# voutcn/megahit

Measured on AMD Instinct MI355X. Metric: M (k+1)-mer edges sorted+counted/sec, sdbg_build k=21, higher is better.
Workload: dtype u32; 1 GPU; read2sdbg (S1+S2) k=21 m=2 no mercy, 10000000 synthetic 150 bp PE reads per GPU (BASELINE configs[1]), inputs resident in HBM, outputs left in HBM; reads_per_gpu=10000000, edges_per_gpu=1290000000, k=21, min_count=2, parallelism=1 GPU, s1_items=1330000000, s2_items=117381042, sdbg_records=59857080

## Files before the change

megahit_amd/csrc/mhx_internal.h:

```cpp
#pragma once
#include <hip/hip_runtime.h>

#include <cstdint>
#include <cstdio>
#include <cstring>
#include <functional>
#include <map>
#include <stdexcept>
#include <string>
#include <vector>

#include "../../include/mhx.h"

namespace mhx {

struct OnesweepLaunch;
void set_error(const char *fmt, ...);

struct Error : std::runtime_error {
  explicit Error(const std::string &s) : std::runtime_error(s) {}
};

#define MHX_HIP(expr)                                                                          \
  do {                                                                                         \
// ... 93 lines not shown
    b.used = bytes;
    return b;
  }
  void prof_begin(const char *name, double bytes);
  void prof_end();
  void prof_collect();
};

#define MHX_LAUNCH(ctx, name, bytes, ...) \
  do {                                    \
    (ctx)->prof_begin(name, bytes);       \
    __VA_ARGS__;                          \
    MHX_HIP(hipGetLastError());           \
    (ctx)->prof_end();                    \
  } while (0)

namespace mhx {

struct SortPass {
  int shift;
  int bits;
  int shift2 = 0;
  int bits2 = 0;
  int prev_lo = -1;
};
struct SortPrep {
  const void *buf = nullptr;
  uint64_t n = 0;
  int hist_passes = 0;
  uint64_t hist_sig = 0;
  std::function<void(const OnesweepLaunch &)> gen;
  uint64_t gen_slots = 0;
  bool gen_var = false;
};
uint32_t *radix_sort(mhx_ctx *c, uint32_t *buf_a, uint32_t *buf_b, uint64_t n, int stride, int key_words,
                     const std::vector<SortPass> &passes, SortPrep *prep = nullptr);
uint32_t *sort_whole_key(mhx_ctx *c, uint32_t *buf_a, uint32_t *buf_b, uint64_t n, int stride, int key_words,
                         const std::vector<SortPass> &passes, SortPrep *prep = nullptr);
std::vector<SortPass> make_passes(int key_words, int lo_bit, int hi_bit);
bool sort_takes_generated_first_pass(const mhx_ctx *c, uint64_t n, int stride, const std::vector<SortPass> &passes);
uint64_t passes_signature(const std::vector<SortPass> &ps);
uint32_t *kmsort_exact(mhx_ctx *c, uint32_t *buf_a, uint32_t *buf_b, uint64_t n, int S, int key_words, SortPrep *prep = nullptr);

void exclusive_scan_u32_u64(mhx_ctx *c, const uint32_t *in, uint64_t *out, uint64_t n, uint64_t *d_total);
void exclusive_scan_u64(mhx_ctx *c, const uint64_t *in, uint64_t *out, uint64_t n, uint64_t *d_total);
void find_group_heads(mhx_ctx *c, const uint32_t *items, uint64_t n, int stride, int cmp_bits,
                      uint64_t *heads, uint64_t *d_count);
uint64_t count_group_heads(mhx_ctx *c, const uint32_t *items, uint64_t n, int stride, int cmp_bits);

struct DigitSpec;
DigitSpec spec_of_pass(const SortPass &ps, int key_words);
std::vector<SortPass> make_passes_ranges(int key_words, const std::vector<std::pair<int, int>> &ranges);
void emit_sdbg(mhx_ctx *c, const uint32_t *sorted, uint64_t n_items, int S, int kw, uint32_t k, int is_seq, mhx_sdbg_result *out, int compact_bits = 0);

void partition_by_owner(mhx_ctx *c, const uint32_t *a, uint32_t *b, uint64_t n, int stride, const uint8_t *lut, int n_parts,
                        uint64_t *counts);
uint64_t s1_extract(mhx_ctx *c, uint32_t k, bool compact, SortPrep *prep, bool defer_items = false, bool filter_in_gen = false);
bool s1_compact(const mhx_ctx *c, uint32_t k, int want_mercy);
bool s1_rank_tagged(const mhx_ctx *c, uint32_t k);
int s1_stride(uint32_t k, bool compact);
struct S1Sources {
  int n = 0;
  std::vector<const uint32_t *> ptr;
  std::vector<uint64_t> count;
  uint32_t *spare = nullptr;
  int pbits = 16;
};
constexpr int kSkmBatch = 8;
constexpr int kSkmSrcMax = 8;
struct SkmFront {
  int n_src;
  const uint4 *src[kSkmSrcMax];
  const uint64_t *src_bounds[kSkmSrcMax];
// ... 138 lines not shown
```

megahit_amd/csrc/s1_skm.hip:

```cpp
#include <cstring>

#include "s1_shared.h"

namespace mhx {

constexpr int kSkmC = 8;
constexpr int kSkmW = 10;
constexpr int kSkmNM = kSkmC + kSkmW - 1;
constexpr int kSkmMinBinBits = 16, kSkmMaxBinBits = 20;

__device__ __forceinline__ uint32_t skm_mix(uint32_t c) {
  uint32_t h = c * 0x9E3779B1u;
  return h ^ (h >> 15);
}
__device__ __forceinline__ uint32_t skm_mix2(uint32_t c) {
  uint32_t h = c * 0x9E3779B1u;
  h ^= h >> 15;
  return h * 0x85EBCA6Bu;
}
__device__ __forceinline__ uint32_t skm_bin_of(uint32_t minh) {
  return (minh ^ (minh >> 16)) * 0x7FEB352Du;
}

template <int NT, int J, bool VAR, bool COUNT = false>
__global__ __launch_bounds__(NT) void k_skm_make(const uint32_t *__restrict__ seq, const uint64_t *__restrict__ start, uint32_t L, uint32_t bpr, uint64_t n_blocks,
                                                 int k, int bin_bits, uint32_t bin_lo, uint32_t bin_hi, int count_items, uint64_t pos_base,
                                                 unsigned long long *__restrict__ hp, uint4 *__restrict__ out, unsigned long long cap,
                                                 unsigned long long *__restrict__ cursor, uint32_t *__restrict__ err, unsigned long long *__restrict__ digit_hist) {
  __shared__ uint32_t sm_scan[NT / kWave + 1];
  __shared__ unsigned long long s_base;
  __shared__ uint32_t dh[3][256];
  __shared__ uint32_t lbin[J * kSkmC][NT];
  __shared__ uint32_t hpl[2][12];
  const int tid = threadIdx.x;
  if (tid < 24) hpl[tid / 12][tid % 12] = 0;
  for (int i = tid; i < 768; i += NT) dh[i >> 8][i & 255] = 0;
  __syncthreads();
  const bool third_digit = bin_bits > 16;
  const int M = k + 1 - (kSkmW - 1);
  const uint32_t mmask = (1u << (2 * M)) - 1u;
  const int K1 = k + 1;
  const unsigned bin_sh = 32u - (unsigned)bin_bits;
  unsigned long long items = 0;
  uint32_t hp_n[2] = {0, 0};
  unsigned long long hp_p[2] = {~0ull, ~0ull};
  for (uint64_t it = blockIdx.x; it * (uint64_t)(NT * J) < n_blocks; it += gridDim.x) {
    uint64_t Wv[J], pos0[J];
    uint32_t smask[J], emask[J];
    uint32_t bflag[J];
#pragma unroll
    for (int j = 0; j < J; ++j) {
      const uint64_t b = it * (uint64_t)(NT * J) + (uint64_t)j * NT + tid;
      smask[j] = 0;
      emask[j] = 0;
      bflag[j] = 0;
      Wv[j] = 0;
      pos0[j] = 0;
      if (b < n_blocks) {
        const uint64_t r = b / bpr;
        const uint32_t q0 = (uint32_t)(b - r * bpr) * kSkmC;
        uint64_t base;
        uint32_t nwin;
        if constexpr (VAR) {
          base = start[r];
          const uint64_t len_r = start[r + 1] - base;
          nwin = len_r >= (uint64_t)K1 ? (uint32_t)(len_r - k) : 0u;
          if (q0 == 0 && nwin && count_items) items += nwin + (COUNT ? 0 : 4);
        } else {
          base = r * L;
// ... 45 lines not shown
                    const unsigned prev_raw = q0 + w == 0 ? kSentinel
                                              : (w == 0 ? (unsigned)((seq[(a - 1) >> 4] >> (30 - 2 * (unsigned)((a - 1) & 15))) & 3u) : (unsigned)(W >> (64 - 2 * w)) & 3u);
                    const unsigned next_raw = q0 + w + 1 == nwin ? kSentinel : (unsigned)(W >> (62 - 2 * (w + K1))) & 3u;
                    const unsigned pv = strand ? comp_or_sentinel(next_raw) : prev_raw, nx = strand ? comp_or_sentinel(prev_raw) : next_raw;
                    atomicAdd(&hpl[cls][0], 1u);
                    if (pv < 4) atomicAdd(&hpl[cls][1 + pv], 1u);
                    if (nx < 4) atomicAdd(&hpl[cls][5 + nx], 1u);
                  } else {
                    ++hp_n[cls];
                    hp_p[cls] = min(hp_p[cls], pos_base + a + (uint64_t)w);
                  }
                }
            }
          }
#pragma unroll
          for (int w = 0; w < kSkmC; ++w)
            if ((uint32_t)w < n_here && !((hm >> w) & 1u) && bins[w] >= bin_lo && bins[w] < bin_hi) km |= 1u << w;
#pragma unroll
          for (int w = 0; w < kSkmC; ++w)
            if (((km >> w) & 1u) && (w == 0 || !((km >> (w - 1)) & 1u) || bins[w] != bins[w > 0 ? w - 1 : 0])) sm |= 1u << w;
          smask[j] = sm;
          emask[j] = km & ((sm >> 1) | ~(km >> 1));
          if constexpr (COUNT) {
            const uint64_t pb = a > 0 ? (uint64_t)((seq[(a - 1) >> 4] >> (30 - 2 * (unsigned)((a - 1) & 15))) & 3u) : 0ull;
            Wv[j] = (W >> 2) | (pb << 62);
            bflag[j] = (q0 == 0 ? 1u : 0u) | (q0 + n_here == nwin ? 2u : 0u) | (n_here << 2);
          } else {
            Wv[j] = W;
          }
          pos0[j] = pos_base + a;
        }
      }
    }
    uint32_t cnt = 0;
#pragma unroll
    for (int j = 0; j < J; ++j) cnt += (uint32_t)__builtin_popcount(smask[j]);
    uint32_t total = 0;
    const uint32_t excl = block_exclusive_sum<uint32_t, NT>(cnt, sm_scan, &total);
    if (tid == 0) s_base = total ? atomicAdd(cursor, (unsigned long long)total) : 0ull;
    __syncthreads();
    const unsigned long long base = s_base;
    if (base + total > cap) {
      if (tid == 0) atomicOr(err, 1u);
      return;
    }
    unsigned long long at = base + excl;
#pragma unroll
    for (int j = 0; j < J; ++j) {
      uint32_t sm = smask[j], em = emask[j];
      while (sm) {
        const int rs = __builtin_ctz(sm), re = __builtin_ctz(em);
        sm &= sm - 1;
        em &= em - 1;
        const int len = re - rs + 1;
        const uint32_t run_bin = lbin[j * kSkmC + rs][tid];
        const uint64_t p = pos0[j] + (uint64_t)rs;
        if constexpr (COUNT) {
          const uint64_t bases = (Wv[j] << (2 * rs)) & (~0ull << (64 - 2 * (K1 + len + 1)));
          const uint32_t n_blk = bflag[j] >> 2;
          const uint32_t fl = ((bflag[j] & 1u) && rs == 0 ? 16u : 0u) | ((bflag[j] & 2u) && (uint32_t)(re + 1) == n_blk ? 8u : 0u);
          out[at++] = make_uint4((run_bin << 8) | ((uint32_t)(p >> 32) << 28) | ((uint32_t)(len - 1) << 5) | fl, (uint32_t)(bases >> 32), (uint32_t)bases, (uint32_t)p);
        } else {
        const uint64_t bases = ((Wv[j] << (2 * rs)) & (~0ull << (64 - 2 * (K1 + len - 1)))) | (uint64_t)(len - 1);
        out[at++] = make_uint4((run_bin << 8) | ((uint32_t)(p >> 32) << 28), (uint32_t)(bases >> 32), (uint32_t)bases, (uint32_t)p);
        }
        atomicAdd(&dh[0][run_bin & 255u], 1u);
        atomicAdd(&dh[1][(run_bin >> 8) & 255u], 1u);
        if (third_digit) atomicAdd(&dh[2][run_bin >> 16], 1u);
      }
    }
  }
  if constexpr (VAR) {
    items = wave_sum(items);
    if ((tid & (kWave - 1)) == 0 && items) atomicAdd(cursor + 3, items);
  }
  if constexpr (COUNT) {
    __syncthreads();
    if (hp && count_items && tid < 24 && hpl[tid / 12][tid % 12]) atomicAdd(hp + 8 + (tid / 12) * 16 + (tid % 12), (unsigned long long)hpl[tid / 12][tid % 12]);
  }
  if (!COUNT && hp && count_items) {
#pragma unroll
    for (int x = 0; x < 2; ++x) {
      const uint32_t n_w = wave_sum(hp_n[x]);
      if (n_w) {
        unsigned long long pmin = hp_p[x];
#pragma unroll
        for (int d = kWave / 2; d > 0; d >>= 1) pmin = min(pmin, (unsigned long long)__shfl_xor((long long)pmin, d, kWave));
        if ((tid & (kWave - 1)) == 0) {
          atomicAdd(hp + x, (unsigned long long)n_w);
          atomicMin(hp + 2 + x, pmin);
        }
      }
    }
  }
  __syncthreads();
  for (int i = tid; i < 768; i += NT)
    if (dh[i >> 8][i & 255]) atomicAdd(&digit_hist[i], (unsigned long long)dh[i >> 8][i & 255]);
}

__global__ void k_skm_hp_publish(const unsigned long long *__restrict__ hp, int k, uint32_t m, uint8_t *__restrict__ solid_bytes,
                                 unsigned long long *__restrict__ hist, uint2 *__restrict__ agg_items, uint64_t *__restrict__ agg_cursor, int agg) {
  if (threadIdx.x || blockIdx.x) return;
// ... 914 lines not shown

bool s1_skm_dist_applies(const mhx_ctx *c, uint32_t k, uint32_t m) {
  const SeqSet &s = c->seqs;
  if (!c->opt("s1_skm", 1) || !c->opt("dist_skm", 1) || !c->global_bases || c->n_parts > kSkmSrcMax || c->filter_on || c->accumulate) return false;
  if (k < 19 || k > 22 || m < 1 || m > 2 || (c->global_bases >> 36)) return false;
  if (!s.n_seqs || s.max_len < k + 1) return false;
  if (!s.fixed_len && (double)s.n_bases * 100.0 < (double)c->opt("s1_var_min_fill", 50) * (double)s.n_seqs * s.max_len) return false;
  if (getenv("MHX_S1_MARK") || !c->opt("dist_sparse_marks", 1)) return false;
  return s1_skm_passes(c, k) == 1;
}

int s1_skm_passes(const mhx_ctx *c, uint32_t k) {
  const SeqSet &s = c->seqs;
  if (const long long f = c->opt("s1_skm_passes", 0)) return (int)std::min<long long>(64, std::max<long long>(1, f));
  const uint64_t n_win = s.n_bases > s.n_seqs * (uint64_t)k ? s.n_bases - s.n_seqs * (uint64_t)k : 0;
  const double need = (double)n_win * (double)std::max<long long>(c->opt("s1_skm_cap_pct", 36), 1) / 100.0 * 32.0;
  const double budget = (double)std::max<long long>(c->opt("s1_skm_pass_gb", 48), 1) * 1e9;
  return (int)std::min(64.0, std::max(1.0, std::ceil(need / budget)));
}

bool s1_skm_front(mhx_ctx *c, uint32_t k, SkmFront *f, int pass, int n_passes, int bin_bits_agreed, bool for_count) {
  SeqSet &s = c->seqs;
  hipStream_t st = c->stream;
  const bool var = s.fixed_len == 0;
  const uint32_t L = var ? s.max_len : s.fixed_len, bpr = (L - k + kSkmC - 1) / kSkmC;
  const uint64_t n_blocks = s.n_seqs * (uint64_t)bpr;
  const uint64_t n_win = var ? (s.n_bases > s.n_seqs * (uint64_t)k ? s.n_bases - s.n_seqs * (uint64_t)k : 0) : s.n_seqs * (uint64_t)(L - k);
  const uint64_t cap_all = n_win * (uint64_t)std::max<long long>(c->opt("s1_skm_cap_pct", 36), 1) / 100;
  const uint64_t cap = std::max<uint64_t>(n_passes > 1 ? cap_all / n_passes + cap_all / n_passes * 15 / 100 : cap_all, 1u << 16);
  int bin_bits = kSkmMinBinBits;
  while (bin_bits < kSkmMaxBinBits && (double)n_win * 0.29 / (double)(1ull << bin_bits) > 8192.0) ++bin_bits;
  if (const long long fb = c->opt("s1_skm_bin_bits", 0)) bin_bits = (int)std::min<long long>(kSkmMaxBinBits, std::max<long long>(8, fb));
  if (bin_bits_agreed > 0) bin_bits = bin_bits_agreed;
  uint4 *buf_a = c->ws("items_a", cap * 16 + 64).as<uint4>();
  uint4 *buf_b = c->ws("items_b", cap * 16 + 64).as<uint4>();
  unsigned long long *cursor = c->ws("skm_cursor", 64).as<unsigned long long>();
  uint32_t *err = reinterpret_cast<uint32_t *>(cursor + 1);
  uint32_t *max_bin = err + 1;
  MHX_HIP(hipMemsetAsync(cursor, 0, 64, st));
  std::vector<SortPass> passes;
  for (int lo = 0; lo < bin_bits; lo += 8) passes.push_back(SortPass{8 + lo, std::min(8, bin_bits - lo), 0, 0, 0});
  unsigned long long *pre_hist = c->ws("sort_pre_hist", (size_t)kMaxFusedPasses * 256 * 8).as<unsigned long long>();
  MHX_HIP(hipMemsetAsync(pre_hist, 0, (size_t)3 * 256 * 8, st));
  constexpr int NT = 512, J = 2;
  const uint64_t cus = c->n_cus > 0 ? (uint64_t)c->n_cus : 256;
  const unsigned grid = (unsigned)std::min<uint64_t>(div_ceil(n_blocks, (uint64_t)NT * J), cus * 8);
  const uint32_t n_bins = 1u << bin_bits;
  const uint32_t bin_lo = (uint32_t)((uint64_t)n_bins * pass / n_passes), bin_hi = (uint32_t)((uint64_t)n_bins * (pass + 1) / n_passes);
  unsigned long long *hp = nullptr;
  if (!c->global_bases && c->opt("s1_skm_hp", 1)) {
    hp = c->ws("skm_hp", 512).as<unsigned long long>();
    if (pass == 0) {
      unsigned long long init[48] = {0};
      init[2] = init[3] = ~0ull;
      MHX_HIP(hipMemcpyAsync(hp, init, sizeof init, hipMemcpyHostToDevice, st));
      MHX_HIP(hipStreamSynchronize(st));
    }
  }
#define MHX_MAKE(VARV, COUNTV)                                                                                                                                   \
  hipLaunchKernelGGL((k_skm_make<NT, J, VARV, COUNTV>), dim3(grid), dim3(NT), 0, st, s.words.as<uint32_t>(), s.start.as<uint64_t>(), L, bpr, n_blocks, (int)k, \
                     bin_bits, bin_lo, bin_hi, pass == 0 ? 1 : 0, c->pos_base, hp, buf_a, (unsigned long long)cap, cursor, err, pre_hist)
  MHX_LAUNCH(c, for_count ? "count_skm_make" : "s1_skm_make", (double)s.n_bases / 4 + (double)n_win * 16 / 3.5, {
    if (var && for_count) MHX_MAKE(true, true);
    else if (var) MHX_MAKE(true, false);
    else if (for_count) MHX_MAKE(false, true);
    else MHX_MAKE(false, false);
  });
#undef MHX_MAKE
  unsigned long long h[4] = {0, 0, 0, 0};
  std::vector<unsigned long long> h_dh(passes.size() * 256);
  MHX_HIP(hipMemcpyAsync(h, cursor, 32, hipMemcpyDeviceToHost, st));
  MHX_HIP(hipMemcpyAsync(h_dh.data(), pre_hist, h_dh.size() * 8, hipMemcpyDeviceToHost, st));
  MHX_HIP(hipStreamSynchronize(st));
  f->n_records = 0;
  f->hp = hp;
  if ((uint32_t)h[1] != 0 || h[0] > cap) return false;
  const uint64_t n = h[0];
  {
    const uint64_t n_bins_pass = std::max<uint64_t>(1, ((1ull << bin_bits) + n_passes - 1) / n_passes);
    const uint64_t limit = std::max<uint64_t>((uint64_t)c->opt("s1_skm_max_bin", 1 << 16), 16 * (n / n_bins_pass + 1));
    bool all = n > 0;
    uint64_t smallest_excess = ~0ull;
    for (size_t p = 0; p < passes.size() && all; ++p) {
      const uint64_t vals = 1ull << passes[p].bits;
      uint64_t mx = 0;
      for (uint64_t d = 0; d < vals; ++d) mx = std::max<uint64_t>(mx, h_dh[p * 256 + d]);
      const uint64_t mean = n / std::max<uint64_t>(1, (p + 1 == passes.size() && n_passes > 1) ? std::max<uint64_t>(1, vals / n_passes) : vals);
      const uint64_t excess = mx > mean ? mx - mean : 0;
      smallest_excess = std::min(smallest_excess, excess);
      all = excess >= limit + limit / 2;
    }
    if (all) {
      f->n_records = n;
      f->max_bin = (uint32_t)std::min<uint64_t>(smallest_excess, 0xFFFFFFFFu);
      return false;
    }
  }
  SortPrep prep;
  prep.buf = buf_a;
  prep.n = n;
  prep.hist_passes = (int)passes.size();
  prep.hist_sig = passes_signature(passes);
  uint32_t *sorted = radix_sort(c, reinterpret_cast<uint32_t *>(buf_a), reinterpret_cast<uint32_t *>(buf_b), n, 4, 1, passes, &prep);
  uint64_t *bounds = c->ws("s1_bucket_bounds", ((size_t)n_bins + 1) * 8 + 64).as<uint64_t>();
  MHX_LAUNCH(c, "s1_skm_bounds", (double)n_bins * 8 * 30,
             hipLaunchKernelGGL(k_skm_bounds, dim3((n_bins + 1 + 255) / 256), dim3(256), 0, st, reinterpret_cast<const uint4 *>(sorted), n, n_bins, bounds, max_bin));
  uint32_t h_max = 0;
  MHX_HIP(hipMemcpyAsync(&h_max, max_bin, 4, hipMemcpyDeviceToHost, st));
  MHX_HIP(hipStreamSynchronize(st));
  f->n_src = 1;
  f->src[0] = reinterpret_cast<const uint4 *>(sorted);
  f->src_bounds[0] = bounds;
  f->spare = sorted == reinterpret_cast<uint32_t *>(buf_a) ? reinterpret_cast<uint32_t *>(buf_b) : reinterpret_cast<uint32_t *>(buf_a);
  f->spare_bytes = cap * 16;
  f->n_records = n;
  f->n_windows = n_win;
  if (pass == 0) f->n_items = var ? h[3] : s.n_seqs * (uint64_t)(L - k + (for_count ? 0 : 4));
  f->n_bins = n_bins;
  f->bin_lo = bin_lo;
  f->bin_hi = bin_hi;
  f->bin_bits = bin_bits;
  f->max_bin = h_max;
  const uint64_t limit = std::max<uint64_t>((uint64_t)c->opt("s1_skm_max_bin", 1 << 16), 16 * (n / (bin_hi - bin_lo) + 1));
  return h_max <= limit;
}

void s1_skm_groups_launch(mhx_ctx *c, bool agg, unsigned grid, const SkmFront &f, uint32_t k, uint32_t m, uint8_t *solid_bytes, unsigned long long *hist,
                          uint2 *agg_raw, uint32_t agg_cap, uint32_t *agg_counts, uint32_t *err, unsigned long long *marks_raw, uint32_t marks_cap,
                          uint32_t *marks_counts) {
  hipStream_t st = c->stream;
  uint32_t *ticket = c->ws("s1_stream_ticket", 64).as<uint32_t>();
  MHX_HIP(hipMemsetAsync(ticket, 0, 4, st));
  const uint32_t nslot = 1u << kSkmLogSlots;
  SkmArgs a{(int)k, m, solid_bytes, hist, agg_raw, agg_cap, agg_counts, err,
            (uint32_t)std::min<long long>(std::max<long long>(c->opt("s1_stream_fill", nslot * 7 / 8), 1), nslot), (int)std::min<long long>(c->opt("s1_stream_probes", 1024), 1024),
            f.bin_lo, f.bin_hi, marks_raw, marks_cap, marks_counts};
  SkmSrcs srcs{};
  srcs.n = f.n_src;
  for (int q = 0; q < f.n_src; ++q) {
    srcs.ptr[q] = f.src[q];
    srcs.bounds[q] = f.src_bounds[q];
  }
  const uint64_t n_bits = c->global_bases ? c->global_bases : c->seqs.n_bases;
  const bool tags = (n_bits >> 32) != 0 || c->opt("s1_skm_tags", 0) != 0;
  const bool deal = c->opt("s1_skm_deal", 1) != 0;
#define MHX_SKM(AGGV, TAGV)                                                                                                  \
  do {                                                                                                                       \
// ... 104 lines not shown
```

megahit_amd/csrc/sort.hip:

```cpp
#include "dev_prims.h"
#include <cstdlib>
#include <cstring>
#include <string>

#include "mhx_internal.h"
#include "sort_digits.h"
#include "sort_kernels.h"

namespace mhx {

template <int S, int NI>
__global__ __launch_bounds__(kSortThreads) void k_radix_hist(const uint32_t *__restrict__ items, uint64_t n, DigitSpec ds,
                                                             uint32_t *__restrict__ hist, uint64_t n_chunks,
                                                             const uint8_t *__restrict__ lut) {
  __shared__ uint32_t h[kSortWaves][256];
  for (int i = threadIdx.x; i < kSortWaves * 256; i += kSortThreads) (&h[0][0])[i] = 0;
  __syncthreads();
  const int w = threadIdx.x / kWave;
  const uint64_t base = (uint64_t)blockIdx.x * SortCfg<S, NI>::kChunk;
  for (int j = 0; j < SortCfg<S, NI>::kChunk / kSortThreads; ++j) {
    uint64_t idx = base + (uint64_t)j * kSortThreads + threadIdx.x;
    if (idx < n) {
      const uint32_t *p = items + idx * S;
      unsigned d;
// ... 192 lines not shown
uint64_t passes_signature(const std::vector<SortPass> &ps) {
  uint64_t h = 1469598103934665603ull;
  for (const SortPass &q : ps)
    for (int v : {q.shift, q.bits, q.shift2, q.bits2}) h = (h ^ (uint64_t)(v + 1)) * 1099511628211ull;
  return h;
}

DigitSpec spec_of_pass(const SortPass &ps, int key_words) {
  DigitSpec ds{key_words - 1 - ps.shift / 32, (unsigned)(ps.shift % 32), (1u << ps.bits) - 1, 0, 0u, 0u, 0u};
  if (ps.bits2) {
    ds.wi2 = key_words - 1 - ps.shift2 / 32;
    ds.bit2 = (unsigned)(ps.shift2 % 32);
    ds.mask2 = (1u << ps.bits2) - 1;
    ds.sh2 = (unsigned)ps.bits;
  }
  if (ps.prev_lo >= 0 && ps.prev_lo < ps.shift && !ps.bits2 && ps.prev_lo / 32 == (ps.shift + ps.bits - 1) / 32) {
    const unsigned hi = (unsigned)(ps.shift % 32), lo = (unsigned)(ps.prev_lo % 32);
    ds.prev_mask = ((1u << hi) - 1u) & ~((1u << lo) - 1u);
  }
  return ds;
}

struct SortEnv {
  bool classic;
  std::string shape;
  int items;
};
static SortEnv sort_env() {
  const char *e = getenv("MHX_SORT"), *sh = getenv("MHX_SORT_SHAPE"), *it = getenv("MHX_SORT_ITEMS");
  return SortEnv{e && !strcmp(e, "classic"), sh ? sh : "", it ? atoi(it) : 0};
}
static void refuse_unconsumed_generator(const SortPrep &prep, const char *who) {
  if (prep.gen) throw Error(std::string(who) + ": the records of this buffer are to be made by a generated first pass, which this sort path cannot run");
}

template <int S, int NI, int UT>
static uint32_t *radix_sort_onesweep(mhx_ctx *c, uint32_t *a, uint32_t *b, uint64_t n, int key_words, const std::vector<SortPass> &passes,
                                     const SortPrep &prep) {
  const int P = (int)passes.size();
  const bool prep_fits = prep.buf == (const void *)a && prep.n == n;
  const bool gen = prep.gen && prep_fits && S == 3 && NI == 8 && UT == 3;
  if (!gen) refuse_unconsumed_generator(prep, "radix sort (chained scan)");
  const uint64_t gen_slots = gen ? std::max<uint64_t>(prep.gen_slots, n) : n;
  const int xcd_units = c->opt("sort_xcd_units", 1) != 0 && c->n_cus >= 192;
  const uint64_t unit = (uint64_t)kSortThreads * NI * UT;
  auto units_of = [&](uint64_t items) { return xcd_units ? (div_ceil(items, unit) + 127) / 128 * 128 : div_ceil(items, unit); };
  const uint64_t n_units = units_of(n), n_units_gen = units_of(gen_slots);
  hipStream_t st = c->stream;
  constexpr bool kCanUt2 = S == 3 && NI == 8 && UT == 3;
  const bool loaded_ut2 = kCanUt2 && c->opt("sort_loaded_ut2", 0) != 0;
  const uint64_t unit2 = (uint64_t)kSortThreads * NI * 2;
  const uint64_t n_units2 = xcd_units ? (div_ceil(n, unit2) + 127) / 128 * 128 : div_ceil(n, unit2);
  const uint64_t n_status = std::max(n_units_gen, loaded_ut2 ? n_units2 : 0);
  unsigned long long *status = c->ws("sort_status", n_status * 256 * 8).as<unsigned long long>();
  unsigned long long *gh = c->ws("sort_ghist", (size_t)2 * kMaxChainedPasses * 256 * 8).as<unsigned long long>();
  unsigned long long *starts = gh + kMaxChainedPasses * 256;
  constexpr int kErrSlot = kMaxChainedPasses * 8;
  uint32_t *tickets = c->ws("sort_tickets", (kErrSlot + 8) * 4).as<uint32_t>();
  MHX_HIP(hipMemsetAsync(status, 0, n_status * 256 * 8, st));
  MHX_HIP(hipMemsetAsync(gh, 0, (size_t)kMaxChainedPasses * 256 * 8, st));
  MHX_HIP(hipMemsetAsync(tickets, 0, (kErrSlot + 8) * 4, st));
  const double bytes = (double)n * S * 4;
  static const std::string nm_hist = "radix_hist_all_" + std::to_string(S * 4) + "B", nm_scat = "radix_scatter_" + std::to_string(S * 4) + "B";
  const unsigned hgrid = (unsigned)std::min<uint64_t>(div_ceil(n, (uint64_t)kSortThreads * 16), 4096);
  std::vector<DigitSpec> all(P);
  for (int p = 0; p < P; ++p) all[p] = spec_of_pass(passes[p], key_words);
  const bool pre = prep_fits && prep.hist_passes == P && P > 0 && P <= kMaxFusedPasses && prep.hist_sig == passes_signature(passes);
  if (gen && !pre) throw Error("radix sort: a generated first pass needs the digit histograms of the plan (pre-hist)");
  if (pre) MHX_HIP(hipMemcpyAsync(gh, c->work["sort_pre_hist"].p, (size_t)P * 256 * 8, hipMemcpyDeviceToDevice, st));
  for (int p0 = 0; p0 < P && !pre; p0 += kMaxFusedPasses) {
    DigitSpecs specs;
    specs.n = std::min(kMaxFusedPasses, P - p0);
    for (int p = 0; p < specs.n; ++p) specs.d[p] = all[p0 + p];
    MHX_LAUNCH(c, nm_hist.c_str(), bytes,
               hipLaunchKernelGGL((k_radix_hist_all<S>), dim3(hgrid), dim3(kSortThreads), 0, st, a, n, specs, gh + (size_t)p0 * 256));
  }
  hipLaunchKernelGGL(k_bin_starts, dim3(P), dim3(256), 0, st, gh, starts);
  constexpr bool kHasUnitRuns = (S <= 3 && NI == 8 && (UT == 3 || UT == 2)) || (S == 4 && NI == 8 && UT == 2) || (S > 4 && NI == 4 && UT == 2);
  const bool unit_runs = kHasUnitRuns && c->opt("sort_unit_runs", 1) != 0;
  const bool rank_uniform = unit_runs && c->opt("sort_rank_uniform", 1) != 0;
  for (int p = 0; p < P; ++p) {
    const int nb = passes[p].bits + passes[p].bits2;
    const int wi = digit_word_of(all[p], nb, 1);
    if (p == 0 && gen) {
      static const std::string nm_gen = nm_scat + "_gen";
      MHX_LAUNCH(c, nm_gen.c_str(), bytes,
                 prep.gen(OnesweepLaunch{(unsigned)n_units_gen, st, b, gen_slots, all[p], nb, starts + p * 256, status, tickets + p * 8,
                                    tickets + kErrSlot, (unsigned long long)(p + 1), xcd_units, unit_runs ? 1 : 0, wi}));
    } else if (unit_runs) {
      if constexpr (kHasUnitRuns) {
#define MHX_U(RANKV, WIV)                                                                                                                      \
  hipLaunchKernelGGL((k_radix_onesweep_u<S, NI, UT, SrcArray<S>, RANKV, WIV>), dim3((unsigned)n_units), dim3(kSortThreads), 0, st, SrcArray<S>{a}, b, \
                     n, all[p], nb, starts + p * 256, status, tickets + p * 8, tickets + kErrSlot, (unsigned long long)(p + 1), xcd_units)
#define MHX_U2(RANKV, WIV)                                                                                                                     \
  hipLaunchKernelGGL((k_radix_onesweep_u<S, NI, 2, SrcArray<S>, RANKV, WIV>), dim3((unsigned)n_units2), dim3(kSortThreads), 0, st, SrcArray<S>{a}, b, \
                     n, all[p], nb, starts + p * 256, status, tickets + p * 8, tickets + kErrSlot, (unsigned long long)(p + 1), xcd_units)
        if constexpr (kCanUt2) {
          if (loaded_ut2 && wi == 0) {
            MHX_LAUNCH(c, nm_scat.c_str(), 2 * bytes, {
              if (rank_uniform && all[p].prev_mask) MHX_U2(2, 0);
              else MHX_U2(0, 0);
            });
            std::swap(a, b);
            continue;
          }
        }
#undef MHX_U2
        MHX_LAUNCH(c, nm_scat.c_str(), 2 * bytes, {
          if (wi == 0 && rank_uniform && all[p].prev_mask) MHX_U(2, 0);
          else if (wi == 0) MHX_U(0, 0);
          else if (wi == 1) MHX_U(0, 1);
          else MHX_U(0, -1);
        });
#undef MHX_U
      }
    } else {
      MHX_LAUNCH(c, nm_scat.c_str(), 2 * bytes,
                 hipLaunchKernelGGL((k_radix_onesweep<S, NI, UT, SrcArray<S>>), dim3((unsigned)n_units), dim3(kSortThreads), 0, st, SrcArray<S>{a}, b, n,
                                    all[p], nb, starts + p * 256, status, tickets + p * 8, tickets + kErrSlot,
                                    (unsigned long long)(p + 1), xcd_units));
    }
// ... 229 lines not shown
    MHX_HIP(hipMemcpyAsync(&starts[p], offs + (uint64_t)p * n_chunks, 8, hipMemcpyDeviceToHost, c->stream));
  MHX_HIP(hipStreamSynchronize(c->stream));
  for (int p = 0; p < n_parts; ++p) counts[p] = starts[p + 1] - starts[p];
}

void partition_by_owner(mhx_ctx *c, const uint32_t *a, uint32_t *b, uint64_t n, int stride, const uint8_t *lut, int n_parts,
                        uint64_t *counts) {
  if (n_parts > 256) throw Error("partition_by_owner: at most 256 owners");
  switch (stride) {
    case 2: return partition_impl<2>(c, a, b, n, lut, n_parts, counts);
    case 3: return partition_impl<3>(c, a, b, n, lut, n_parts, counts);
    case 4: return partition_impl<4>(c, a, b, n, lut, n_parts, counts);
    case 6: return partition_impl<6>(c, a, b, n, lut, n_parts, counts);
    case 8: return partition_impl<8>(c, a, b, n, lut, n_parts, counts);
    case 10: return partition_impl<10>(c, a, b, n, lut, n_parts, counts);
    case 12: return partition_impl<12>(c, a, b, n, lut, n_parts, counts);
    case 14: return partition_impl<14>(c, a, b, n, lut, n_parts, counts);
    case 16: return partition_impl<16>(c, a, b, n, lut, n_parts, counts);
    case 18: return partition_impl<18>(c, a, b, n, lut, n_parts, counts);
    case 20: return partition_impl<20>(c, a, b, n, lut, n_parts, counts);
    default: throw Error("partition_by_owner: unsupported record stride");
  }
}

bool sort_takes_generated_first_pass(const mhx_ctx *c, uint64_t n, int stride, const std::vector<SortPass> &passes) {
  (void)c;
  const SortEnv env = sort_env();
  if (env.classic) return false;
  if ((!env.shape.empty() && env.shape != "8x3") || (env.items && env.items != default_items<3>())) return false;
  return stride == 3 && n > 0 && passes.size() <= (size_t)kMaxChainedPasses && passes.size() <= (size_t)kMaxFusedPasses &&
         div_ceil(n, (uint64_t)kSortThreads * 8) < (1ull << 31);
}

uint32_t *radix_sort(mhx_ctx *c, uint32_t *a, uint32_t *b, uint64_t n, int stride, int key_words,
                     const std::vector<SortPass> &passes, SortPrep *prep_io) {
  SortPrep prep;
  if (prep_io) std::swap(prep, *prep_io);
  switch (stride) {
    case 2: return radix_sort_impl<2>(c, a, b, n, key_words, passes, prep);
    case 3: return radix_sort_impl<3>(c, a, b, n, key_words, passes, prep);
    case 4: return radix_sort_impl<4>(c, a, b, n, key_words, passes, prep);
    case 6: return radix_sort_impl<6>(c, a, b, n, key_words, passes, prep);
    case 8: return radix_sort_impl<8>(c, a, b, n, key_words, passes, prep);
    case 10: return radix_sort_impl<10>(c, a, b, n, key_words, passes, prep);
    case 12: return radix_sort_impl<12>(c, a, b, n, key_words, passes, prep);
    case 14: return radix_sort_impl<14>(c, a, b, n, key_words, passes, prep);
    case 16: return radix_sort_impl<16>(c, a, b, n, key_words, passes, prep);
    case 18: return radix_sort_impl<18>(c, a, b, n, key_words, passes, prep);
    case 20: return radix_sort_impl<20>(c, a, b, n, key_words, passes, prep);
    default: throw Error("radix_sort: unsupported record stride");
  }
}

}
```

megahit_amd/csrc/sort_kernels.h:

```cpp
#pragma once
#include "dev_prims.h"
#include "sort_digits.h"

namespace mhx {

constexpr int kSortThreads = 256;
constexpr int kSortWaves = kSortThreads / kWave;

template <int S>
constexpr int default_items() {
  return (S <= 4) ? 4 : (S <= 8 ? 8 : (S <= 12 ? 5 : (S <= 16 ? 4 : 3)));
}
template <int S, int ITEMS>
struct SortCfg {
  static constexpr int kItems = ITEMS;
  static constexpr int kTile = kSortThreads * kItems;
  static constexpr int kTilesPerChunk = (16384 / kTile) > 4 ? (16384 / kTile) : 4;
  static constexpr int kChunk = kTile * kTilesPerChunk;
};

template <int S>
struct Rec {
  uint32_t w[S];
};
// ... 47 lines not shown
__device__ __forceinline__ unsigned rec_digit2(const Rec<S> &r, const DigitSpec &ds) {
  unsigned d = rec_digit<S>(r, ds.wi1, ds.bit1, ds.mask1);
  if (ds.mask2) d |= rec_digit<S>(r, ds.wi2, ds.bit2, ds.mask2) << ds.sh2;
  return d;
}
__device__ __forceinline__ unsigned mem_digit(const uint32_t *p, int wi, unsigned bit, unsigned mask) {
  uint64_t v = p[wi];
  if (bit + (32 - __builtin_clz(mask)) > 32 && wi > 0) v |= (uint64_t)p[wi - 1] << 32;
  return (unsigned)(v >> bit) & mask;
}


template <int S>
struct SrcArray {
  const uint32_t *in;
  static constexpr bool kMayDrop = false;
  __device__ __forceinline__ bool is_record(const Rec<S> &) const { return true; }
  template <int NI>
  __device__ __forceinline__ void get(uint64_t first, uint64_t n, Rec<S> (&rec)[NI]) const {
#pragma unroll
    for (int j = 0; j < NI; ++j) {
      const uint64_t gi = first + (uint64_t)j * kWave;
      if (gi < n) load_rec<S>(in + gi * S, rec[j]);
    }
  }
  template <int NI>
  __device__ __forceinline__ uint64_t index(uint64_t tile_base, int w, int lane, int j) const {
    return tile_base + (uint64_t)(w * (kWave * NI) + j * kWave + lane);
  }
  template <int NI, int UT>
  __device__ __forceinline__ void get_unit(uint64_t unit_base, int w, int lane, uint64_t n, Rec<S> (&rec)[UT][NI]) const {
#pragma unroll
    for (int t = 0; t < UT; ++t) get<NI>(unit_base + (uint64_t)t * (kSortThreads * NI) + (uint64_t)(w * (kWave * NI) + lane), n, rec[t]);
  }
};

constexpr unsigned long long kStValMask = (1ull << 56) - 1;

template <int S, int NI, int UT, class Src, bool ANY_ORDER = false>
__global__ __launch_bounds__(kSortThreads) void k_radix_onesweep(Src src, uint32_t *__restrict__ out, uint64_t n,
                                                                 DigitSpec ds, int nbits, const unsigned long long *__restrict__ bin_start,
                                                                 unsigned long long *__restrict__ status, uint32_t *__restrict__ ticket,
                                                                 uint32_t *__restrict__ err, unsigned long long tag, int xcd_units) {
  constexpr int kTile = kSortThreads * NI;
  __shared__ __attribute__((aligned(16))) uint32_t stage[kTile * S];
  __shared__ uint32_t wave_cnt[kSortWaves][256];
  __shared__ long long g_off[256];
  __shared__ uint64_t g_base[256];
  __shared__ uint32_t sm_scan[kSortThreads / kWave + 1];
  __shared__ uint32_t s_unit;

  const int tid = threadIdx.x, w = tid / kWave, lane = tid & (kWave - 1);
  const uint64_t lanemask_lt = (1ull << lane) - 1;
  if (tid == 0) {
    if (xcd_units) {
      const uint32_t cls = blockIdx.x & 7u, tk = atomicAdd(ticket + cls, 1u);
      s_unit = ((tk >> 4) * 8 + cls) * 16 + (tk & 15u);
    } else {
      s_unit = atomicAdd(ticket, 1u);
    }
  }
#pragma unroll
  for (int i = 0; i < kSortWaves; ++i) wave_cnt[i][tid] = 0;
  __syncthreads();
  const uint64_t unit = s_unit;
  const uint64_t unit_base = unit * (uint64_t)(kTile * UT);
// ... 304 lines not shown
```

Baseline: 52360 M edges/s.

## Fuse first radix digit scatter into skm_make via per-digit split ranges

The super-k-mer make kernel now partitions records by their lowest bin digit while emitting them. It counts digits per block, reserves space from per-digit global cursors into fixed-capacity ranges, stages records in shared memory and writes them digit-grouped. The radix sort then skips its first digit pass and reads these ranges unit by unit through a new split source that pads unfilled slots. This removes one full read/write pass over the records. In exchange it enlarges buffers, adds shared-memory atomics and staging, and falls back to a full rerun of the make kernel if any digit range overflows.

Result: faster. 54640 M edges/s, median of 6 (+4.4%).

```diff
diff --git a/megahit_amd/csrc/mhx_internal.h b/megahit_amd/csrc/mhx_internal.h
--- a/megahit_amd/csrc/mhx_internal.h
+++ b/megahit_amd/csrc/mhx_internal.h
@@ -149,6 +149,9 @@
   std::function<void(const OnesweepLaunch &)> gen;
   uint64_t gen_slots = 0;
   bool gen_var = false;
+  const unsigned long long *split_fill = nullptr, *split_ubase = nullptr;
+  uint64_t split_range_cap = 0, split_units = 0;
+  int hist_first = 0;
 };
 uint32_t *radix_sort(mhx_ctx *c, uint32_t *buf_a, uint32_t *buf_b, uint64_t n, int stride, int key_words,
                      const std::vector<SortPass> &passes, SortPrep *prep = nullptr);
@@ -156,6 +159,8 @@
                          const std::vector<SortPass> &passes, SortPrep *prep = nullptr);
 std::vector<SortPass> make_passes(int key_words, int lo_bit, int hi_bit);
 bool sort_takes_generated_first_pass(const mhx_ctx *c, uint64_t n, int stride, const std::vector<SortPass> &passes);
+bool sort_takes_split_first_pass(const mhx_ctx *c, const std::vector<SortPass> &passes);
+constexpr uint64_t kSortSplitUnit = 4096;
 uint64_t passes_signature(const std::vector<SortPass> &ps);
 uint32_t *kmsort_exact(mhx_ctx *c, uint32_t *buf_a, uint32_t *buf_b, uint64_t n, int S, int key_words, SortPrep *prep = nullptr);
 
diff --git a/megahit_amd/csrc/s1_skm.hip b/megahit_amd/csrc/s1_skm.hip
--- a/megahit_amd/csrc/s1_skm.hip
+++ b/megahit_amd/csrc/s1_skm.hip
@@ -22,12 +22,18 @@
   return (minh ^ (minh >> 16)) * 0x7FEB352Du;
 }
 
-template <int NT, int J, bool VAR, bool COUNT = false>
+constexpr int kSkmStage = 2560;
+template <int NT, int J, bool VAR, bool COUNT = false, bool SPLIT = false>
 __global__ __launch_bounds__(NT) void k_skm_make(const uint32_t *__restrict__ seq, const uint64_t *__restrict__ start, uint32_t L, uint32_t bpr, uint64_t n_blocks,
                                                  int k, int bin_bits, uint32_t bin_lo, uint32_t bin_hi, int count_items, uint64_t pos_base,
                                                  unsigned long long *__restrict__ hp, uint4 *__restrict__ out, unsigned long long cap,
-                                                 unsigned long long *__restrict__ cursor, uint32_t *__restrict__ err, unsigned long long *__restrict__ digit_hist) {
+                                                 unsigned long long *__restrict__ cursor, uint32_t *__restrict__ err, unsigned long long *__restrict__ digit_hist,
+                                                 unsigned long long range_cap, unsigned long long *__restrict__ split_cur, uint32_t stage_n) {
+  constexpr long long kNoRoom = -0x7FFFFFFFFFFFFFFFll - 1;
   __shared__ uint32_t sm_scan[NT / kWave + 1];
+  __shared__ uint4 stage[SPLIT ? kSkmStage : 1];
+  __shared__ uint32_t dcnt[SPLIT ? 256 : 1], dpos[SPLIT ? 256 : 1];
+  __shared__ long long goff[SPLIT ? 256 : 1];
   __shared__ unsigned long long s_base;
   __shared__ uint32_t dh[3][256];
   __shared__ uint32_t lbin[J * kSkmC][NT];
@@ -35,6 +41,7 @@
   const int tid = threadIdx.x;
   if (tid < 24) hpl[tid / 12][tid % 12] = 0;
   for (int i = tid; i < 768; i += NT) dh[i >> 8][i & 255] = 0;
+  if (SPLIT && tid < 256) dcnt[tid] = 0;
   __syncthreads();
   const bool third_digit = bin_bits > 16;
   const int M = k + 1 - (kSkmW - 1);
@@ -146,6 +153,83 @@
         }
       }
     }
+    auto rec_of = [&](int j, int rs, int re, uint32_t run_bin) -> uint4 {
+      const int len = re - rs + 1;
+      const uint64_t p = pos0[j] + (uint64_t)rs;
+      if constexpr (COUNT) {
+        const uint64_t bases = (Wv[j] << (2 * rs)) & (~0ull << (64 - 2 * (K1 + len + 1)));
+        const uint32_t n_blk = bflag[j] >> 2;
+        const uint32_t fl = ((bflag[j] & 1u) && rs == 0 ? 16u : 0u) | ((bflag[j] & 2u) && (uint32_t)(re + 1) == n_blk ? 8u : 0u);
+        return make_uint4((run_bin << 8) | ((uint32_t)(p >> 32) << 28) | ((uint32_t)(len - 1) << 5) | fl, (uint32_t)(bases >> 32), (uint32_t)bases, (uint32_t)p);
+      } else {
+        const uint64_t bases = ((Wv[j] << (2 * rs)) & (~0ull << (64 - 2 * (K1 + len - 1)))) | (uint64_t)(len - 1);
+        return make_uint4((run_bin << 8) | ((uint32_t)(p >> 32) << 28), (uint32_t)(bases >> 32), (uint32_t)bases, (uint32_t)p);
+      }
+    };
+    auto walk = [&](auto &&fn) {
+#pragma unroll
+      for (int j = 0; j < J; ++j) {
+        uint32_t sm = smask[j], em = emask[j];
+        while (sm) {
+          const int rs = __builtin_ctz(sm), re = __builtin_ctz(em);
+          sm &= sm - 1;
+          em &= em - 1;
+          fn(j, rs, re, lbin[j * kSkmC + rs][tid]);
+        }
+      }
+    };
+    if constexpr (SPLIT) {
+      walk([&](int, int, int, uint32_t run_bin) {
+        atomicAdd(&dcnt[run_bin & 255u], 1u);
+        atomicAdd(&dh[1][(run_bin >> 8) & 255u], 1u);
+        if (third_digit) atomicAdd(&dh[2][run_bin >> 16], 1u);
+      });
+      __syncthreads();
+      const uint32_t c = tid < 256 ? dcnt[tid] : 0u;
+      const uint32_t inc = wave_inclusive_sum(c);
+      if (tid < 256 && (tid & (kWave - 1)) == kWave - 1) sm_scan[tid / kWave] = inc;
+      __syncthreads();
+      uint32_t total = 0, start = inc - c;
+#pragma unroll
+      for (int i = 0; i < 256 / kWave; ++i) {
+        const uint32_t t = sm_scan[i];
+        if (i < tid / kWave) start += t;
+        total += t;
+      }
+      if (tid < 256) {
+        long long off = kNoRoom;
+        if (c) {
+          const unsigned long long gb = atomicAdd(&split_cur[tid], (unsigned long long)c);
+          if (gb + c <= range_cap) off = (long long)((unsigned long long)tid * range_cap + gb) - (long long)start;
+          else atomicOr(err, 2u);
+          dh[0][tid] += c;
+        }
+        goff[tid] = off;
+        dpos[tid] = start;
+        dcnt[tid] = 0;
+      }
+      __syncthreads();
+      const bool direct = total > stage_n;
+      walk([&](int j, int rs, int re, uint32_t run_bin) {
+        const uint32_t d = run_bin & 255u;
+        const uint32_t pos = atomicAdd(&dpos[d], 1u);
+        const uint4 rec = rec_of(j, rs, re, run_bin);
+        if (direct) {
+          const long long off = goff[d];
+          if (off != kNoRoom) out[off + (long long)pos] = rec;
+        } else {
+          stage[pos] = rec;
+        }
+      });
+      if (!direct) {
+        __syncthreads();
+        for (uint32_t i = tid; i < total; i += NT) {
+          const uint4 rec = stage[i];
+          const long long off = goff[(rec.x >> 8) & 255u];
+          if (off != kNoRoom) out[off + (long long)i] = rec;
+        }
+      }
+    } else {
     uint32_t cnt = 0;
 #pragma unroll
     for (int j = 0; j < J; ++j) cnt += (uint32_t)__builtin_popcount(smask[j]);
@@ -159,29 +243,12 @@
       return;
     }
     unsigned long long at = base + excl;
-#pragma unroll
-    for (int j = 0; j < J; ++j) {
-      uint32_t sm = smask[j], em = emask[j];
-      while (sm) {
-        const int rs = __builtin_ctz(sm), re = __builtin_ctz(em);
-        sm &= sm - 1;
-        em &= em - 1;
-        const int len = re - rs + 1;
-        const uint32_t run_bin = lbin[j * kSkmC + rs][tid];
-        const uint64_t p = pos0[j] + (uint64_t)rs;
-        if constexpr (COUNT) {
-          const uint64_t bases = (Wv[j] << (2 * rs)) & (~0ull << (64 - 2 * (K1 + len + 1)));
-          const uint32_t n_blk = bflag[j] >> 2;
-          const uint32_t fl = ((bflag[j] & 1u) && rs == 0 ? 16u : 0u) | ((bflag[j] & 2u) && (uint32_t)(re + 1) == n_blk ? 8u : 0u);
-          out[at++] = make_uint4((run_bin << 8) | ((uint32_t)(p >> 32) << 28) | ((uint32_t)(len - 1) << 5) | fl, (uint32_t)(bases >> 32), (uint32_t)bases, (uint32_t)p);
-        } else {
-        const uint64_t bases = ((Wv[j] << (2 * rs)) & (~0ull << (64 - 2 * (K1 + len - 1)))) | (uint64_t)(len - 1);
-        out[at++] = make_uint4((run_bin << 8) | ((uint32_t)(p >> 32) << 28), (uint32_t)(bases >> 32), (uint32_t)bases, (uint32_t)p);
-        }
-        atomicAdd(&dh[0][run_bin & 255u], 1u);
-        atomicAdd(&dh[1][(run_bin >> 8) & 255u], 1u);
-        if (third_digit) atomicAdd(&dh[2][run_bin >> 16], 1u);
-      }
+    walk([&](int j, int rs, int re, uint32_t run_bin) {
+      out[at++] = rec_of(j, rs, re, run_bin);
+      atomicAdd(&dh[0][run_bin & 255u], 1u);
+      atomicAdd(&dh[1][(run_bin >> 8) & 255u], 1u);
+      if (third_digit) atomicAdd(&dh[2][run_bin >> 16], 1u);
+    });
     }
   }
   if constexpr (VAR) {
@@ -1162,46 +1229,68 @@
   while (bin_bits < kSkmMaxBinBits && (double)n_win * 0.29 / (double)(1ull << bin_bits) > 8192.0) ++bin_bits;
   if (const long long fb = c->opt("s1_skm_bin_bits", 0)) bin_bits = (int)std::min<long long>(kSkmMaxBinBits, std::max<long long>(8, fb));
   if (bin_bits_agreed > 0) bin_bits = bin_bits_agreed;
-  uint4 *buf_a = c->ws("items_a", cap * 16 + 64).as<uint4>();
-  uint4 *buf_b = c->ws("items_b", cap * 16 + 64).as<uint4>();
+  std::vector<SortPass> passes;
+  for (int lo = 0; lo < bin_bits; lo += 8) passes.push_back(SortPass{8 + lo, std::min(8, bin_bits - lo), 0, 0, 0});
+  const std::vector<SortPass> passes_rest(passes.begin() + (passes.empty() ? 0 : 1), passes.end());
+  bool split = c->opt("s1_skm_split", 1) != 0 && passes.size() >= 2 && sort_takes_split_first_pass(c, passes_rest);
+  const uint64_t cap_split = std::max<uint64_t>(cap, 1u << 20), range_cap = cap_split / 256 / kSortSplitUnit * kSortSplitUnit;
+  const uint64_t cap_alloc = split ? cap_split : cap;
+  uint4 *buf_a = c->ws("items_a", cap_alloc * 16 + 64).as<uint4>();
+  uint4 *buf_b = c->ws("items_b", cap_alloc * 16 + 64).as<uint4>();
   unsigned long long *cursor = c->ws("skm_cursor", 64).as<unsigned long long>();
   uint32_t *err = reinterpret_cast<uint32_t *>(cursor + 1);
   uint32_t *max_bin = err + 1;
-  MHX_HIP(hipMemsetAsync(cursor, 0, 64, st));
-  std::vector<SortPass> passes;
-  for (int lo = 0; lo < bin_bits; lo += 8) passes.push_back(SortPass{8 + lo, std::min(8, bin_bits - lo), 0, 0, 0});
+  unsigned long long *split_cur = split ? c->ws("skm_split_cursors", (256 + 257) * 8).as<unsigned long long>() : nullptr;
+  const uint32_t stage_n = (uint32_t)std::min<long long>(std::max<long long>(c->opt("s1_skm_split_stage", kSkmStage), 0), kSkmStage);
   unsigned long long *pre_hist = c->ws("sort_pre_hist", (size_t)kMaxFusedPasses * 256 * 8).as<unsigned long long>();
-  MHX_HIP(hipMemsetAsync(pre_hist, 0, (size_t)3 * 256 * 8, st));
   constexpr int NT = 512, J = 2;
   const uint64_t cus = c->n_cus > 0 ? (uint64_t)c->n_cus : 256;
   const unsigned grid = (unsigned)std::min<uint64_t>(div_ceil(n_blocks, (uint64_t)NT * J), cus * 8);
   const uint32_t n_bins = 1u << bin_bits;
   const uint32_t bin_lo = (uint32_t)((uint64_t)n_bins * pass / n_passes), bin_hi = (uint32_t)((uint64_t)n_bins * (pass + 1) / n_passes);
   unsigned long long *hp = nullptr;
-  if (!c->global_bases && c->opt("s1_skm_hp", 1)) {
-    hp = c->ws("skm_hp", 512).as<unsigned long long>();
-    if (pass == 0) {
-      unsigned long long init[48] = {0};
-      init[2] = init[3] = ~0ull;
-      MHX_HIP(hipMemcpyAsync(hp, init, sizeof init, hipMemcpyHostToDevice, st));
-      MHX_HIP(hipStreamSynchronize(st));
-    }
-  }
-#define MHX_MAKE(VARV, COUNTV)                                                                                                                                   \
-  hipLaunchKernelGGL((k_skm_make<NT, J, VARV, COUNTV>), dim3(grid), dim3(NT), 0, st, s.words.as<uint32_t>(), s.start.as<uint64_t>(), L, bpr, n_blocks, (int)k, \
-                     bin_bits, bin_lo, bin_hi, pass == 0 ? 1 : 0, c->pos_base, hp, buf_a, (unsigned long long)cap, cursor, err, pre_hist)
-  MHX_LAUNCH(c, for_count ? "count_skm_make" : "s1_skm_make", (double)s.n_bases / 4 + (double)n_win * 16 / 3.5, {
-    if (var && for_count) MHX_MAKE(true, true);
-    else if (var) MHX_MAKE(true, false);
-    else if (for_count) MHX_MAKE(false, true);
-    else MHX_MAKE(false, false);
-  });
+  if (!c->global_bases && c->opt("s1_skm_hp", 1)) hp = c->ws("skm_hp", 512).as<unsigned long long>();
+  unsigned long long hp_init[48] = {0};
+  hp_init[2] = hp_init[3] = ~0ull;
+  unsigned long long h[4] = {0, 0, 0, 0};
+  std::vector<unsigned long long> h_dh(passes.size() * 256), h_fill(256);
+#define MHX_MAKE(VARV, COUNTV, SPLITV)                                                                                                                                   \
+  hipLaunchKernelGGL((k_skm_make<NT, J, VARV, COUNTV, SPLITV>), dim3(grid), dim3(NT), 0, st, s.words.as<uint32_t>(), s.start.as<uint64_t>(), L, bpr, n_blocks, (int)k, \
+                     bin_bits, bin_lo, bin_hi, pass == 0 ? 1 : 0, c->pos_base, hp, buf_a, (unsigned long long)cap, cursor, err, pre_hist,                            \
+                     (unsigned long long)range_cap, split_cur, stage_n)
+  auto make = [&](bool split_now) {
+    MHX_HIP(hipMemsetAsync(cursor, 0, 64, st));
+    MHX_HIP(hipMemsetAsync(pre_hist, 0, (size_t)3 * 256 * 8, st));
+    if (split_now) MHX_HIP(hipMemsetAsync(split_cur, 0, 256 * 8, st));
+    if (hp && pass == 0) MHX_HIP(hipMemcpyAsync(hp, hp_init, sizeof hp_init, hipMemcpyHostToDevice, st));
+    MHX_LAUNCH(c, for_count ? "count_skm_make" : "s1_skm_make", (double)s.n_bases / 4 + (double)n_win * 16 / 3.5, {
+      if (split_now) {
+        if (var && for_count) MHX_MAKE(true, true, true);
+        else if (var) MHX_MAKE(true, false, true);
+        else if (for_count) MHX_MAKE(false, true, true);
+        else MHX_MAKE(false, false, true);
+      } else {
+        if (var && for_count) MHX_MAKE(true, true, false);
+        else if (var) MHX_MAKE(true, false, false);
+        else if (for_count) MHX_MAKE(false, true, false);
+        else MHX_MAKE(false, false, false);
+      }
+    });
+    MHX_HIP(hipMemcpyAsync(h, cursor, 32, hipMemcpyDeviceToHost, st));
+    MHX_HIP(hipMemcpyAsync(h_dh.data(), pre_hist, h_dh.size() * 8, hipMemcpyDeviceToHost, st));
+    if (split_now) MHX_HIP(hipMemcpyAsync(h_fill.data(), split_cur, 256 * 8, hipMemcpyDeviceToHost, st));
+    MHX_HIP(hipStreamSynchronize(st));
+  };
+  make(split);
+  if (split && ((uint32_t)h[1] & 2u)) {
+    split = false;
+    make(false);
+  }
 #undef MHX_MAKE
-  unsigned long long h[4] = {0, 0, 0, 0};
-  std::vector<unsigned long long> h_dh(passes.size() * 256);
-  MHX_HIP(hipMemcpyAsync(h, cursor, 32, hipMemcpyDeviceToHost, st));
-  MHX_HIP(hipMemcpyAsync(h_dh.data(), pre_hist, h_dh.size() * 8, hipMemcpyDeviceToHost, st));
-  MHX_HIP(hipStreamSynchronize(st));
+  if (split) {
+    h[0] = 0;
+    for (int d = 0; d < 256; ++d) h[0] += h_fill[d];
+  }
   f->n_records = 0;
   f->hp = hp;
   if ((uint32_t)h[1] != 0 || h[0] > cap) return false;
@@ -1226,12 +1315,24 @@
       return false;
     }
   }
+  const std::vector<SortPass> &sort_passes = split ? passes_rest : passes;
   SortPrep prep;
   prep.buf = buf_a;
   prep.n = n;
-  prep.hist_passes = (int)passes.size();
-  prep.hist_sig = passes_signature(passes);
-  uint32_t *sorted = radix_sort(c, reinterpret_cast<uint32_t *>(buf_a), reinterpret_cast<uint32_t *>(buf_b), n, 4, 1, passes, &prep);
+  prep.hist_passes = (int)sort_passes.size();
+  prep.hist_sig = passes_signature(sort_passes);
+  std::vector<unsigned long long> h_ubase(257, 0);
+  if (split) {
+    for (int d = 0; d < 256; ++d) h_ubase[d + 1] = h_ubase[d] + div_ceil((uint64_t)h_fill[d], kSortSplitUnit);
+    unsigned long long *ubase = split_cur + 256;
+    MHX_HIP(hipMemcpyAsync(ubase, h_ubase.data(), 257 * 8, hipMemcpyHostToDevice, st));
+    prep.split_fill = split_cur;
+    prep.split_ubase = ubase;
+    prep.split_units = h_ubase[256];
+    prep.split_range_cap = range_cap;
+    prep.hist_first = 1;
+  }
+  uint32_t *sorted = radix_sort(c, reinterpret_cast<uint32_t *>(buf_a), reinterpret_cast<uint32_t *>(buf_b), n, 4, 1, sort_passes, &prep);
   uint64_t *bounds = c->ws("s1_bucket_bounds", ((size_t)n_bins + 1) * 8 + 64).as<uint64_t>();
   MHX_LAUNCH(c, "s1_skm_bounds", (double)n_bins * 8 * 30,
              hipLaunchKernelGGL(k_skm_bounds, dim3((n_bins + 1 + 255) / 256), dim3(256), 0, st, reinterpret_cast<const uint4 *>(sorted), n, n_bins, bounds, max_bin));
@@ -1242,7 +1343,7 @@
   f->src[0] = reinterpret_cast<const uint4 *>(sorted);
   f->src_bounds[0] = bounds;
   f->spare = sorted == reinterpret_cast<uint32_t *>(buf_a) ? reinterpret_cast<uint32_t *>(buf_b) : reinterpret_cast<uint32_t *>(buf_a);
-  f->spare_bytes = cap * 16;
+  f->spare_bytes = cap_alloc * 16;
   f->n_records = n;
   f->n_windows = n_win;
   if (pass == 0) f->n_items = var ? h[3] : s.n_seqs * (uint64_t)(L - k + (for_count ? 0 : 4));
diff --git a/megahit_amd/csrc/sort.hip b/megahit_amd/csrc/sort.hip
--- a/megahit_amd/csrc/sort.hip
+++ b/megahit_amd/csrc/sort.hip
@@ -248,6 +248,7 @@
 }
 static void refuse_unconsumed_generator(const SortPrep &prep, const char *who) {
   if (prep.gen) throw Error(std::string(who) + ": the records of this buffer are to be made by a generated first pass, which this sort path cannot run");
+  if (prep.split_fill) throw Error(std::string(who) + ": the records of this buffer lie in ranges split by an earlier digit, which this sort path cannot read");
 }
 
 template <int S, int NI, int UT>
@@ -256,8 +257,12 @@
   const int P = (int)passes.size();
   const bool prep_fits = prep.buf == (const void *)a && prep.n == n;
   const bool gen = prep.gen && prep_fits && S == 3 && NI == 8 && UT == 3;
-  if (!gen) refuse_unconsumed_generator(prep, "radix sort (chained scan)");
-  const uint64_t gen_slots = gen ? std::max<uint64_t>(prep.gen_slots, n) : n;
+  constexpr bool kCanSplit = S == 4 && NI == 8 && UT == 2;
+  static_assert(!kCanSplit || (uint64_t)kSortThreads * NI * UT == kSortSplitUnit, "a unit of the split pass");
+  const bool split = kCanSplit && !prep.gen && prep.split_fill && prep.split_ubase && prep_fits && c->opt("sort_unit_runs", 1) != 0 &&
+                     prep.split_range_cap > 0 && prep.split_range_cap % kSortSplitUnit == 0;
+  if (!gen && !split) refuse_unconsumed_generator(prep, "radix sort (chained scan)");
+  const uint64_t gen_slots = gen ? std::max<uint64_t>(prep.gen_slots, n) : (split ? prep.split_units * kSortSplitUnit : n);
   const int xcd_units = c->opt("sort_xcd_units", 1) != 0 && c->n_cus >= 192;
   const uint64_t unit = (uint64_t)kSortThreads * NI * UT;
   auto units_of = [&](uint64_t items) { return xcd_units ? (div_ceil(items, unit) + 127) / 128 * 128 : div_ceil(items, unit); };
@@ -283,7 +288,10 @@
   for (int p = 0; p < P; ++p) all[p] = spec_of_pass(passes[p], key_words);
   const bool pre = prep_fits && prep.hist_passes == P && P > 0 && P <= kMaxFusedPasses && prep.hist_sig == passes_signature(passes);
   if (gen && !pre) throw Error("radix sort: a generated first pass needs the digit histograms of the plan (pre-hist)");
-  if (pre) MHX_HIP(hipMemcpyAsync(gh, c->work["sort_pre_hist"].p, (size_t)P * 256 * 8, hipMemcpyDeviceToDevice, st));
+  if (split && !pre) throw Error("radix sort: a split first pass needs the digit histograms of the plan (pre-hist)");
+  if (pre)
+    MHX_HIP(hipMemcpyAsync(gh, static_cast<const unsigned long long *>(c->work["sort_pre_hist"].p) + (size_t)prep.hist_first * 256, (size_t)P * 256 * 8,
+                           hipMemcpyDeviceToDevice, st));
   for (int p0 = 0; p0 < P && !pre; p0 += kMaxFusedPasses) {
     DigitSpecs specs;
     specs.n = std::min(kMaxFusedPasses, P - p0);
@@ -303,6 +311,19 @@
       MHX_LAUNCH(c, nm_gen.c_str(), bytes,
                  prep.gen(OnesweepLaunch{(unsigned)n_units_gen, st, b, gen_slots, all[p], nb, starts + p * 256, status, tickets + p * 8,
                                     tickets + kErrSlot, (unsigned long long)(p + 1), xcd_units, unit_runs ? 1 : 0, wi}));
+    } else if (p == 0 && split) {
+      if constexpr (kCanSplit) {
+#define MHX_US(RANKV, WIV)                                                                                                                        \
+  hipLaunchKernelGGL((k_radix_onesweep_u<S, NI, UT, SrcSplit<S>, RANKV, WIV>), dim3((unsigned)n_units_gen), dim3(kSortThreads), 0, st,            \
+                     SrcSplit<S>{a, prep.split_fill, prep.split_ubase, prep.split_range_cap}, b, gen_slots, all[p], nb, starts + p * 256, status, tickets + p * 8, \
+                     tickets + kErrSlot, (unsigned long long)(p + 1), xcd_units)
+        MHX_LAUNCH(c, nm_scat.c_str(), 2 * bytes, {
+          if (wi == 0 && rank_uniform && all[p].prev_mask) MHX_US(2, 0);
+          else if (wi == 0) MHX_US(0, 0);
+          else MHX_US(0, -1);
+        });
+#undef MHX_US
+      }
     } else if (unit_runs) {
       if constexpr (kHasUnitRuns) {
 #define MHX_U(RANKV, WIV)                                                                                                                      \
@@ -598,6 +619,13 @@
          div_ceil(n, (uint64_t)kSortThreads * 8) < (1ull << 31);
 }
 
+bool sort_takes_split_first_pass(const mhx_ctx *c, const std::vector<SortPass> &passes) {
+  const SortEnv env = sort_env();
+  if (env.classic || c->opt("sort_unit_runs", 1) == 0) return false;
+  if ((!env.shape.empty() && env.shape != "8x2") || (env.items && env.items != default_items<4>())) return false;
+  return !passes.empty() && passes.size() <= (size_t)kMaxChainedPasses && passes.size() <= (size_t)kMaxFusedPasses;
+}
+
 uint32_t *radix_sort(mhx_ctx *c, uint32_t *a, uint32_t *b, uint64_t n, int stride, int key_words,
                      const std::vector<SortPass> &passes, SortPrep *prep_io) {
   SortPrep prep;
diff --git a/megahit_amd/csrc/sort_kernels.h b/megahit_amd/csrc/sort_kernels.h
--- a/megahit_amd/csrc/sort_kernels.h
+++ b/megahit_amd/csrc/sort_kernels.h
@@ -103,6 +103,49 @@
   __device__ __forceinline__ void get_unit(uint64_t unit_base, int w, int lane, uint64_t n, Rec<S> (&rec)[UT][NI]) const {
 #pragma unroll
     for (int t = 0; t < UT; ++t) get<NI>(unit_base + (uint64_t)t * (kSortThreads * NI) + (uint64_t)(w * (kWave * NI) + lane), n, rec[t]);
+  }
+};
+template <int S>
+struct SrcSplit {
+  const uint32_t *in;
+  const unsigned long long *fill;
+  const unsigned long long *ubase;
+  uint64_t range_cap;
+  static constexpr bool kMayDrop = true;
+  __device__ __forceinline__ bool is_record(const Rec<S> &r) const { return (r.w[0] & 7u) == 0u; }
+  template <int NI>
+  __device__ __forceinline__ uint64_t index(uint64_t tile_base, int w, int lane, int j) const {
+    return tile_base + (uint64_t)(w * (kWave * NI) + j * kWave + lane);
+  }
+  template <int NI, int UT>
+  __device__ __forceinline__ void get_unit(uint64_t unit_base, int w, int lane, uint64_t n, Rec<S> (&rec)[UT][NI]) const {
+    constexpr uint64_t kUnit = (uint64_t)kSortThreads * NI * UT;
+    const uint64_t u = unit_base / kUnit;
+    uint64_t first = 0, end = 0;
+#pragma unroll
+    for (int q = 0; q < 4; ++q) {
+      const int d = q * kWave + lane;
+      const uint64_t lo = ubase[d], hi = ubase[d + 1];
+      const uint64_t m = __ballot(lo <= u && u < hi);
+      if (m) {
+        const int src = __builtin_ctzll(m);
+        const uint64_t dd = (uint64_t)(q * kWave + src);
+        const uint64_t lo_d = (uint64_t)__shfl((long long)lo, src, kWave);
+        uint64_t filled = fill[dd];
+        if (filled > range_cap) filled = range_cap;
+        first = dd * range_cap + (u - lo_d) * kUnit;
+        end = dd * range_cap + filled;
+      }
+    }
+#pragma unroll
+    for (int t = 0; t < UT; ++t)
+#pragma unroll
+      for (int j = 0; j < NI; ++j) {
+        const uint64_t gi = first + (uint64_t)t * (kSortThreads * NI) + (uint64_t)(w * (kWave * NI) + j * kWave + lane);
+#pragma unroll
+        for (int i = 0; i < S; ++i) rec[t][j].w[i] = 0xFFFFFFFFu;
+        if (gi < end) load_rec<S>(in + gi * S, rec[t][j]);
+      }
   }
 };
 
```
